# Robin-Lenoir/replication-social-bank-runs

Hardware: AMD Instinct MI355X
Metric: equilibria solved/sec on β×u grid (FP64) (higher is better)
Workload: dtype f64; 1 GPU; fig5_beta_u_sweep_2048x2048_per_gpu (BASELINE config 3); n_beta_per_gpu=2048, n_u=2048, early_exit=False, parallelism=beta-column shards x1, beta_axis_columns=2048, pipelined=True

## Files before the change

include/sbr.h:

```cpp
#ifndef SBR_H
#define SBR_H

#include <stdint.h>

#include "sbr_status.h"

#ifdef __cplusplus
extern "C" {
#endif

#define SBR_OK 0
#define SBR_EARG (-1)
#define SBR_EDEVICE (-2)
#define SBR_ENOMEM (-3)

typedef struct sbr_ctx sbr_ctx;

typedef struct {
    double ode_reltol;
    double ode_abstol;
    int64_t ode_maxiters;
    int32_t bisect_max_iters;
    int32_t early_exit_nan_run;
    int32_t knot_capacity;
    int32_t hetero_max_iters;
    int32_t flags;
    int32_t pad;
    double xi_guess;
} sbr_opts;

#define SBR_FLAG_EXHAUSTIVE 0x1
#define SBR_FLAG_READY_SWEEP 0x2
#define SBR_FLAG_RCCL_GATHER 0x4
#define SBR_FLAG_XI_GUESS 0x8
#define SBR_FLAG_DIAG_STOP_AFTER_BUFFER 0x100
#define SBR_FLAG_DIAG_STOP_AFTER_BISECT 0x200
#define SBR_FLAG_DIAG_COUNT_AW_BLOCKS 0x400
#define SBR_FLAG_DIAG_SOCIAL_PROF 0x800
#define SBR_FLAG_DIAG_NO_AW_WINDOW 0x1000
#define SBR_FLAG_HETERO_WIDE 0x2000

#define SBR_HETERO_MAX_K 16

typedef struct {
    double* xi;
    double* tau_in_unc;
    double* tau_out_unc;
    double* aw_max;
    double* tol;
    uint32_t* status;
    int32_t* iters;
} sbr_result_soa;

void sbr_default_opts(sbr_opts* o);

int sbr_init(int device, sbr_ctx** ctx);
int sbr_free(sbr_ctx* ctx);
const char* sbr_last_error(const sbr_ctx* ctx);

int sbr_init_multi(int n_gpus, const int* devices, sbr_ctx** ctx);
int sbr_multi_size(const sbr_ctx* ctx);
sbr_ctx* sbr_multi_child(sbr_ctx* ctx, int rank);

// ... 171 lines not shown
```

replication-social-bank-runs_amd/csrc/sbr_capi_baseline.hip:

```cpp
#include "sbr_hostio.h"

using namespace sbr_capi;

namespace sbr_capi {

void free_learn(sbr_ctx* c, int slot)
{
    sbr::LearnBufs& L = c->LW[slot];
    free_dev(L.t, L.G, L.hr, L.hrI, L.n_knots, L.n_tau, L.n_le, L.status, L.n_accept, L.n_reject);
    L = sbr::LearnBufs{};
    c->ws_beta[slot] = c->ws_cap[slot] = 0;
}

size_t learn_ld(size_t cap) { return ((cap + 15) & ~(size_t)15) + 16; }

int ensure_learn(sbr_ctx* c, size_t n_beta, size_t cap, int slot, bool hri)
{
    if (n_beta <= c->ws_beta[slot] && cap == c->ws_cap[slot] && (!hri || c->LW[slot].hrI)) return SBR_OK;
    free_learn(c, slot);
    sbr::LearnBufs& L = c->LW[slot];
    const size_t ld = learn_ld(cap);
    const size_t slab = n_beta * ld * sizeof(double);
    const int rc = alloc_dev(c, {{L.t, slab}, {L.G, slab}, {L.hr, slab}, {L.hrI, hri ? slab : 0},
                                 {L.n_knots, n_beta * 4}, {L.n_tau, n_beta * 4}, {L.n_le, n_beta * 4},
// ... 38 lines not shown
    free_econ(c);
    const int rc = alloc_dev(c, {{c->ec_hr, rows * ld * sizeof(double)}, {c->ec_cnt, rows * 3 * sizeof(int32_t)}});
    if (rc) return rc;
    c->ec_rows = rows;
    c->ec_ld = ld;
    return SBR_OK;
}

}

namespace {

int32_t stop_after_eta(const sbr_opts& o)
{
    const double e = 2.220446049250313e-16;
    return (o.ode_reltol == e && o.ode_abstol == e && o.ode_maxiters >= SBR_DEFAULT_ODE_MAXITERS) ? 1 : 0;
}

int launch_eq(sbr_ctx* c, hipStream_t s, const sbr::LearnBufs& L, const double* eta, const double* t_end,
              const double* u, int64_t n_beta, int64_t n_u, double kappa, const sbr_opts& o,
              const sbr::ResultSoA& out, double* aw_path, int group = 1, bool timed = true)
{
    sbr::EqArgs ea{kappa, (int32_t)n_u, o.bisect_max_iters, c->lds_cap_b, aw_path,
                   (o.flags & SBR_FLAG_EXHAUSTIVE) ? 1 : 0, (o.flags >> 8) & 0x17};
    ea.group = group;
    hipEvent_t t0 = timed ? tstart(c, s) : nullptr;
    if (aw_path && n_beta == 1 && n_u == 1) {
        ea.lds_cap = c->lds_cap;
        HIP_TRY(c, sbr::launch_point_coop(L, eta, t_end, u, ea, out, s), SBR_EDEVICE);
        tend(c, s, 1, t0);
        return SBR_OK;
    }
    HIP_TRY(c, sbr::launch_equilibrium(L, eta, t_end, u, ea, out, (int)n_beta, s), SBR_EDEVICE);
    tend(c, s, 1, t0);
    return SBR_OK;
}

#ifndef SBR_BATCH_LEARN_WAVES
#define SBR_BATCH_LEARN_WAVES 768
#endif
#ifndef SBR_BATCH_EQ_COLS
#define SBR_BATCH_EQ_COLS 4096
#endif
struct BatchPlan {
    int64_t L = 1;
    int64_t E = 1;
    int nslot = 1;
// ... 85 lines not shown
        c->rq_cap = need;
    }
    return SBR_OK;
}

int run_baseline_ready(sbr_ctx* c, hipStream_t s, const double* beta, const double* eta, const double* t_end,
                       const double* u, int64_t n_beta, int64_t n_u, double kappa, const sbr_opts& o,
                       sbr::LearnArgs la, const sbr::ResultSoA& out)
{
    const int tiles = (int)((n_u + kReadyTileU - 1) / kReadyTileU);
    int32_t* q = c->rq;
    HIP_TRY(c, hipEventRecord(c->ev_rin, s), SBR_EDEVICE);
    HIP_TRY(c, hipStreamWaitEvent(c->rs_learn, c->ev_rin, 0), SBR_EDEVICE);
    HIP_TRY(c, hipMemsetAsync(q, 0, (4 + 2 * (size_t)n_beta) * 4, c->rs_learn), SBR_EDEVICE);
    HIP_TRY(c, hipEventRecord(c->ev_rq, c->rs_learn), SBR_EDEVICE);
    HIP_TRY(c, hipStreamWaitEvent(c->rs_eq, c->ev_rq, 0), SBR_EDEVICE);
    la.fuse_hazard = 0;
    la.ready_tail = q + 2;
    la.ready_q = q + 4;
    hipEvent_t t0 = tstart(c, c->rs_learn);
    HIP_TRY(c, sbr::launch_learn_logistic(beta, eta, t_end, la, c->LW[0], c->rs_learn), SBR_EDEVICE);
    tend(c, c->rs_learn, 0, t0);
    sbr::EqArgs ea{kappa, (int32_t)n_u, o.bisect_max_iters, c->lds_cap_b, nullptr,
                   (o.flags & SBR_FLAG_EXHAUSTIVE) ? 1 : 0, (o.flags >> 8) & 0x17};
    sbr::ReadyArgs ra{q, q + 4, q + 4 + n_beta, (int32_t)(n_beta * tiles), tiles, kReadyTileU, kReadySpin};
    hipEvent_t t1 = tstart(c, c->rs_eq);
    HIP_TRY(c, sbr::launch_eq_ready(c->LW[0], beta, eta, t_end, u, la, ea, ra, out, 0, c->rs_eq), SBR_EDEVICE);
    tend(c, c->rs_eq, 1, t1);
    HIP_TRY(c, hipEventRecord(c->ev_rl, c->rs_learn), SBR_EDEVICE);
    HIP_TRY(c, hipEventRecord(c->ev_re, c->rs_eq), SBR_EDEVICE);
    HIP_TRY(c, hipStreamWaitEvent(s, c->ev_rl, 0), SBR_EDEVICE);
    HIP_TRY(c, hipStreamWaitEvent(s, c->ev_re, 0), SBR_EDEVICE);
    HIP_TRY(c, sbr::launch_ready_fail(q + 1, out, n_beta * n_u, s), SBR_EDEVICE);
    return SBR_OK;
}

int run_baseline(sbr_ctx* c, hipStream_t s, const double* beta, const double* eta, const double* t_end, double x0,
                 const double* u, int64_t n_beta, int64_t n_u, double p, double kappa, double lambda,
                 const sbr_opts& o, const sbr::ResultSoA& out, double* aw_path)
{
    int rc = ensure_learn(c, (size_t)n_beta, (size_t)o.knot_capacity);
    if (rc) return rc;
    c->last_slot = 0;
    c->last_off = 0;
    sbr::LearnArgs la{x0, o.ode_reltol, o.ode_abstol, p, lambda, o.ode_maxiters, (int32_t)n_beta, stop_after_eta(o), 0};
    c->rs_used = !aw_path && n_beta >= 64 && (o.flags & SBR_FLAG_READY_SWEEP) &&
                 ensure_ready(c, (size_t)n_beta) == SBR_OK;
// ... 14 lines not shown
        const int64_t wk = waves >> (kSweepChunks - k);
        lo[k] = std::min<int64_t>(n_beta, std::max<int64_t>(wk * 64, (int64_t)k * 64));
    }
    lo[1] = std::min<int64_t>(lo[2] - 64, std::max<int64_t>(64, (waves / kSweepFront) * 64));
    HIP_TRY(c, hipEventRecord(c->ev_in, s), SBR_EDEVICE);
    hipEvent_t t0 = tstart(c, s);
    c->ck_start = c->timing ? t0 : nullptr;
    c->ck_ev.assign(c->timing ? 2 * kSweepChunks : 0, nullptr);
    for (int k = 0; k < kSweepChunks; k++) {
        hipStream_t ls = c->lstream[k];
        const int64_t c0 = lo[k], nb = lo[k + 1] - lo[k];
        HIP_TRY(c, hipStreamWaitEvent(ls, c->ev_in, 0), SBR_EDEVICE);
        if (nb <= 0) continue;
        sbr::LearnArgs lk = la;
        lk.n_beta = (int32_t)nb;
        const sbr::LearnBufs Lk = learn_rows(c->LW[0], (size_t)c0);
        HIP_TRY(c, sbr::launch_learn_logistic(beta + c0, eta + c0, t_end + c0, lk, Lk, ls), SBR_EDEVICE);
        if (c->timing) {
            c->ck_ev[2 * k] = next_event(c);
            if (c->ck_ev[2 * k]) (void)hipEventRecord(c->ck_ev[2 * k], ls);
        }
        HIP_TRY(c, hipEventRecord(c->ev_learned[k], ls), SBR_EDEVICE);
        sbr::EqArgs ea{kappa, (int32_t)n_u, o.bisect_max_iters, c->lds_cap_b, nullptr,
                       (o.flags & SBR_FLAG_EXHAUSTIVE) ? 1 : 0, (o.flags >> 8) & 0x17};
        HIP_TRY(c, sbr::launch_equilibrium(Lk, eta + c0, t_end + c0, u, ea, result_rows(out, (size_t)(c0 * n_u)),
                                           (int)nb, ls), SBR_EDEVICE);
        if (c->timing) {
            c->ck_ev[2 * k + 1] = next_event(c);
            if (c->ck_ev[2 * k + 1]) (void)hipEventRecord(c->ck_ev[2 * k + 1], ls);
        }
        HIP_TRY(c, hipEventRecord(c->ev_eq[k], ls), SBR_EDEVICE);
    }
    for (int k = 0; k < kSweepChunks; k++)
        if (lo[k + 1] > lo[k]) HIP_TRY(c, hipStreamWaitEvent(s, c->ev_learned[k], 0), SBR_EDEVICE);
    hipEvent_t t1 = tstart(c, s);
    tend(c, s, 0, t0);
    for (int k = 0; k < kSweepChunks; k++)
        if (lo[k + 1] > lo[k]) HIP_TRY(c, hipStreamWaitEvent(s, c->ev_eq[k], 0), SBR_EDEVICE);
    tend(c, s, 1, t1);
    return SBR_OK;
}

size_t point_bytes(size_t cap) { return 4 * cap * sizeof(double) + 6 * sizeof(int32_t); }

int run_points(sbr_ctx* c, hipStream_t s, const double* beta, const double* eta, const double* t_end, double x0,
               const double* u, const double* p, const double* kappa, const double* lambda, int64_t n,
               const sbr_opts& o, const sbr::ResultSoA& out)
// ... 53 lines not shown
    const double budget = c->ec_budget > 0 ? (double)c->ec_budget : 0.4 * (double)(freeb + held);
    const double left = budget - (double)n_beta * (double)point_bytes(cap);
    int64_t per = left > 0.0 ? (int64_t)std::min(left / ((double)n_beta * (double)econ_class_bytes(cap)), 65535.0) : 1;
    per = std::max<int64_t>(1, std::min<int64_t>(per, n_class));
    int rc = ensure_learn(c, (size_t)n_beta, cap);
    if (rc) return rc;
    c->last_slot = 0;
    c->last_off = 0;
    c->rs_used = false;
    const sbr::LearnBufs& L = c->LW[0];
    for (;;) {
        rc = ensure_econ(c, (size_t)(per * n_beta), (size_t)L.cap);
        if (rc == SBR_OK) break;
        free_econ(c);
        if (per == 1) return rc;
        (void)hipGetLastError();
        per = (per + 1) / 2;
    }
    sbr::LearnArgs la{x0, o.ode_reltol, o.ode_abstol, 0.0, 0.0, o.ode_maxiters, (int32_t)n_beta, stop_after_eta(o), 0};
    hipEvent_t t0 = tstart(c, s);
    HIP_TRY(c, sbr::launch_learn_kernel(beta, eta, t_end, la, L, s, 1), SBR_EDEVICE);
    tend(c, s, 0, t0);
    sbr::EqArgs ea{0.0, (int32_t)(n_kappa * n_u), o.bisect_max_iters, rates ? c->lds_cap : c->lds_cap_b, nullptr,
                   (o.flags & SBR_FLAG_EXHAUSTIVE) ? 1 : 0, (o.flags >> 8) & 0x17};
    const sbr::InterestEconArgs ie{rates ? rates->r : nullptr, rates ? rates->delta : nullptr,
                                   (int32_t)(rates ? rates->n : 0), o.ode_reltol, o.ode_abstol, o.ode_maxiters,
                                   rates ? rates->steps : nullptr};
    t0 = tstart(c, s);
    int launches = 0;
    for (int64_t g0 = 0; g0 < n_class; g0 += per) {
        const int64_t ng = std::min<int64_t>(per, n_class - g0);
        const size_t rows = (size_t)(per * n_beta);
        const sbr::EconArgs e{p, lambda, kappa, (int32_t)n_p, (int32_t)n_lambda, (int32_t)n_kappa, (int32_t)n_u,
                              (int32_t)n_beta, (int32_t)g0, (int32_t)ng, c->ec_hr, c->ec_cnt, c->ec_cnt + rows,
                              (uint32_t*)(c->ec_cnt + 2 * rows)};
        HIP_TRY(c, sbr::launch_hazard_econ(beta, eta, la, L, e, s), SBR_EDEVICE);
        if (rates) HIP_TRY(c, sbr::launch_interest_econ(L, eta, t_end, u, ea, e, ie, out, s), SBR_EDEVICE);
        else HIP_TRY(c, sbr::launch_equilibrium_econ(L, eta, t_end, u, ea, e, out, s), SBR_EDEVICE);
        launches += 3;
    }
    tend(c, s, 1, t0, launches);
    return SBR_OK;
}

int econ_checks(sbr_ctx* c, const sbr_opts* opts, double x0, int64_t n_beta, int64_t n_u, int64_t n_p,
                int64_t n_lambda, int64_t n_kappa)
{
// ... 1 lines not shown
    if (!c) return SBR_EARG;
    const int64_t lim = 1 << 30;
    if (n_beta <= 0 || n_u <= 0 || n_p <= 0 || n_lambda <= 0 || n_kappa <= 0 || n_beta > lim || n_u > lim ||
        n_p > lim || n_lambda > lim || n_kappa > lim || n_p * n_lambda > lim || n_kappa * n_u > lim)
        return fail(c, SBR_EARG, "grid size");
    if (!(x0 >= 0.0)) return fail(c, SBR_EARG, "ArgumentError: x0");
    return SBR_OK;
}

int run_interest(sbr_ctx* c, hipStream_t s, const double* beta, const double* eta, const double* t_end, double x0,
                 const double* u, int64_t n_beta, int64_t n_u, double p, double kappa, double lambda, double r,
                 double delta, const sbr_opts& o, const sbr::ResultSoA& out, int64_t* steps, double* aw_path = nullptr,
                 double* v_path = nullptr, int32_t* v_count = nullptr)
{
    int rc = ensure_learn(c, (size_t)n_beta, (size_t)o.knot_capacity);
    if (rc) return rc;
    c->last_slot = 0;
    c->last_off = 0;
    sbr::LearnArgs la{x0, o.ode_reltol, o.ode_abstol, p, lambda, o.ode_maxiters, (int32_t)n_beta, stop_after_eta(o), 0};
    hipEvent_t t0 = tstart(c, s);
    HIP_TRY(c, sbr::launch_learn_logistic(beta, eta, t_end, la, c->LW[0], s), SBR_EDEVICE);
    tend(c, s, 0, t0);
    sbr::EqArgs ea{kappa, (int32_t)n_u, o.bisect_max_iters, c->lds_cap, aw_path,
                   (o.flags & SBR_FLAG_EXHAUSTIVE) ? 1 : 0, (o.flags >> 8) & 0x17};
    sbr::InterestArgs ia{r, delta, o.ode_reltol, o.ode_abstol, o.ode_maxiters, steps, v_path, v_count};
    t0 = tstart(c, s);
    HIP_TRY(c, sbr::launch_interest(c->LW[0], eta, t_end, u, ea, ia, out, (int)n_beta, s), SBR_EDEVICE);
    tend(c, s, 1, t0);
    return SBR_OK;
}

bool interest_valid(double r, double delta) { return r >= 0.0 && delta > 0.0 && r < delta; }

}

extern "C" {

int sbr_sweep_baseline_dev(sbr_ctx* c, void* stream, const double* beta, const double* eta, const double* t_end,
                           double x0, const double* u, int64_t n_beta, int64_t n_u, double p, double kappa,
                           double lambda, const sbr_opts* opts, sbr_result_soa* out)
{
    if (int rc = refuse_guess(c, opts)) return rc;
    SBR_SINGLE_DEVICE(c);
    if (!c || !has_fields(out)) return SBR_EARG;
    if (n_beta <= 0 || n_u <= 0 || n_beta > (1 << 30) || n_u > (1 << 30)) return fail(c, SBR_EARG, "grid size");
    if (!scalars_valid(x0, p, kappa, lambda)) return fail(c, SBR_EARG, "ArgumentError: x0/p/kappa/lambda");
    if (hipSetDevice(c->device) != hipSuccess) return fail(c, SBR_EDEVICE, "hipSetDevice");
// ... 643 lines not shown
```

replication-social-bank-runs_amd/csrc/sbr_capi_knots.hip:

```cpp
#include "sbr_hostio.h"

using namespace sbr_capi;

namespace {

struct KnotLayout {
    size_t sc, tg, hr, u, res, bytes;
    KnotLayout(size_t ck, size_t cu)
    {
        sc = 64;
        tg = 128;
        hr = tg + 24 * ck;
        u = hr + 8 * (ck + 8);
        res = u + 8 * (cu + 8);
        bytes = res + 8 * (6 * cu + 3 * (ck + 1)) + 256;
    }
};

int ensure_knots(sbr_ctx* c, size_t n, size_t n_u)
{
    if (n <= c->kn_cap_k && n_u <= c->kn_cap_u) return SBR_OK;
    size_t ck = c->kn_cap_k > 4096 ? c->kn_cap_k : 4096, cu = c->kn_cap_u > 64 ? c->kn_cap_u : 64;
    while (ck < n) ck *= 2;
    while (cu < n_u) cu *= 2;
// ... 246 lines not shown
            double* hs = (double*)(H + K.sc);
            hs[0] = beta;
            hs[1] = eta;
            memcpy(H + K.tg, t, (size_t)n * 8);
            memcpy(H + K.tg + (size_t)n * 8, G, (size_t)n * 8);
            if (pdf) memcpy(H + K.tg + (size_t)n * 16, pdf, (size_t)n * 8);
            HIP_TRY(c, hipMemcpyAsync(D, H, K.tg + (size_t)n * (pdf ? 24 : 16), hipMemcpyHostToDevice, s), SBR_EDEVICE);
            sbr::LearnArgs la{0.0, o.ode_reltol, o.ode_abstol, p, lambda, o.ode_maxiters, 1, 0, 0, nullptr, nullptr};
            la.pdf = pdf ? dtg + 2 * n : nullptr;
            HIP_TRY(c, sbr::launch_hazard(dsc, dsc + 1, la, L, 1, s), SBR_EDEVICE);
            if (ntau > 0)
                HIP_TRY(c, hipMemcpyAsync(H + K.hr, D + K.hr, (size_t)ntau * 8, hipMemcpyDeviceToHost, s), SBR_EDEVICE);
            HIP_TRY(c, hipMemcpyAsync(H, D, 32, hipMemcpyDeviceToHost, s), SBR_EDEVICE);
        }
        const size_t nu = (size_t)n_u;
        if (n_u == 1) {
            double* z = c->kn_zc;
            double* zd = c->kn_zc_dev;
            z[0] = t_end;
            z[1] = u[0];
            const sbr::ResultSoA r{zd + 2, zd + 3, zd + 4, zd + 5, zd + 6, (uint32_t*)(zd + 7), (int32_t*)(zd + 7) + 1};
            double* zp = zd + 16;
            sbr::EqArgs ea{kappa, 1, o.bisect_max_iters, c->lds_cap, want_aw ? zp : nullptr,
                           (o.flags & SBR_FLAG_EXHAUSTIVE) ? 1 : 0, (o.flags >> 8) & 0x17,
                           want_aw ? zp + ntau : nullptr, want_aw ? zp + 2 * ntau : nullptr, 1, dres};
            if (o.flags & SBR_FLAG_XI_GUESS) ea.xi_guess = o.xi_guess;
            HIP_TRY(c, sbr::launch_point_coop(L, dsc + 1, zd, zd + 1, ea, r, s), SBR_EDEVICE);
        } else {
            double* hu = (double*)(H + K.u);
            hu[0] = t_end;
            memcpy(hu + 1, u, nu * 8);
            HIP_TRY(c, hipMemcpyAsync(du, hu, (nu + 1) * 8, hipMemcpyHostToDevice, s), SBR_EDEVICE);
            const sbr::ResultSoA r{dres, dres + nu, dres + 2 * nu, dres + 3 * nu, dres + 4 * nu,
                                   (uint32_t*)(dres + 5 * nu), (int32_t*)(dres + 5 * nu) + nu};
            if ((o.flags & SBR_FLAG_XI_GUESS) && o.xi_guess == o.xi_guess) {
                sbr::EqArgs ea{kappa, 1, o.bisect_max_iters, c->lds_cap, nullptr,
                               (o.flags & SBR_FLAG_EXHAUSTIVE) ? 1 : 0, (o.flags >> 8) & 0x17, nullptr, nullptr, 1};
                ea.xi_guess = o.xi_guess;
                HIP_TRY(c, sbr::launch_point_coop(L, dsc + 1, du, du + 1, ea, r, s, (int)nu), SBR_EDEVICE);
            } else {
                sbr::EqArgs ea{kappa, (int32_t)n_u, o.bisect_max_iters, c->lds_cap_b, nullptr,
                               (o.flags & SBR_FLAG_EXHAUSTIVE) ? 1 : 0, (o.flags >> 8) & 0x17, nullptr, nullptr, 1};
                HIP_TRY(c, sbr::launch_equilibrium(L, dsc + 1, du, du + 1, ea, r, 1, s, n <= c->lds_cap_b ? 1 : 2),
                        SBR_EDEVICE);
            }
            HIP_TRY(c, hipMemcpyAsync(H + K.res, D + K.res, res_bytes, hipMemcpyDeviceToHost, s), SBR_EDEVICE);
        }
        HIP_TRY(c, hipStreamSynchronize(s), SBR_EDEVICE);
        return SBR_OK;
    });
    if (rc) return rc;
    if (!hit) {
        const int32_t* hc = (const int32_t*)H;
        if (hc[1] != (int32_t)ntau) return fail(c, SBR_EDEVICE, "hazard grid length mismatch");
        c->kn_t.assign(t, t + n);
        c->kn_G.assign(G, G + n);
        if (pdf) c->kn_pdf.assign(pdf, pdf + n);
        else c->kn_pdf.clear();
        const double* hh = (const double*)(H + K.hr);
        c->kn_hr.assign(hh, hh + ntau);
        memcpy(c->kn_key, key, sizeof key);
        c->kn_n = n;
        c->kn_m = (int32_t)m;
        c->kn_ntau = (int32_t)ntau;
        c->kn_valid = true;
// ... 50 lines not shown
```

replication-social-bank-runs_amd/csrc/sbr_eq_column_body.h:

```cpp
{
    const int n = L.n_knots[b], ntau = L.n_tau[b], nle = L.n_le[b];
    const uint32_t lst = L.status[b];
    const size_t row = (size_t)b * (size_t)L.cap;
    const double* __restrict__ gT = L.t + row;
    const double* __restrict__ gG = L.G + row;
    const double* __restrict__ gH = L.hr + row;
    constexpr int NS = INTEREST ? 3 : 2;
    const bool fits = n <= a.lds_cap && (!INTEREST || ntau <= a.lds_cap);
    if ((MODE == 1 && !fits) || (MODE == 2 && fits)) return;
    double* sT = smem;
    double* sG = smem + a.lds_cap;
    double* sH = INTEREST ? smem + 2 * a.lds_cap : nullptr;
    const double* __restrict__ cH = INTEREST ? sH : gH;
    const int nsum = (a.lds_cap >> 6) + 1, nsum8 = (a.lds_cap >> 3) + 1;
    double* hmax = smem + NS * a.lds_cap;
    double* hmin = hmax + nsum;
    double* pmc = hmin + nsum;
    double* smc = pmc + nsum8;
    double* hpm = smc + nsum8;
    double* hpn = hpm + nsum;
    double* hsm = hpn + nsum;
    double* hsn = hsm + nsum;
    const int nbh_s = (ntau + 63) >> 6;
    __shared__ int eq_next;
    __shared__ int s_nonmono;
    __shared__ int s_noscan;
    __shared__ int s_near1;
    __shared__ int s_ndec;
    __shared__ unsigned long long s_maxdec;
    __shared__ double s_thalf;
    __shared__ int s_wb;
    __shared__ unsigned long long s_dmax;
    if (threadIdx.x == 0) { eq_next = 0; s_nonmono = 0; s_noscan = 0; s_near1 = 0; s_ndec = 0; s_maxdec = 0; s_thalf = NAN; s_wb = 0x7fffffff; s_dmax = 0; }
    if (fits) {
        for (int i = threadIdx.x; i < n; i += BLOCK) { sT[i] = gT[i]; sG[i] = gG[i]; }
        if (INTEREST)
            for (int i = threadIdx.x; i < ntau; i += BLOCK) sH[i] = gH[i];
    }
    __syncthreads();
    Summ S{nullptr, nullptr, nullptr, nullptr, false, (double)NAN, false, 0.0, false, 2, nullptr, nullptr, nullptr,
           nullptr, 0};
    if (fits && !a.exhaustive) {
        const int nbh = (ntau + 63) >> 6, nbg = (n + 7) >> 3;
        const int nq = nbh << 3;
        for (int bk = threadIdx.x; bk < nq + nbg; bk += BLOCK) {
            if (bk < nq) {
                double mx = -INFINITY, mn = INFINITY;
                const int i0 = bk << 3;
                double h[8];
#pragma unroll
                for (int k = 0; k < 8; k++) h[k] = i0 + k < ntau ? cH[i0 + k] : -INFINITY;
#pragma unroll
                for (int k = 0; k < 8; k++) {
                    if (i0 + k >= ntau) continue;
                    if (h[k] > mx) mx = h[k];
                    mn = (h[k] != h[k]) ? -INFINITY : (h[k] < mn ? h[k] : mn);
// ... 15 lines not shown
                double prev = g > 0 ? sG[(g << 3) - 1] : -INFINITY;
                bool mono = true, nan = false;
                int ndec = 0;
                double maxdec = 0.0;
                for (int i = g << 3; i < e; i++) {
                    const double v = sG[i];
                    if (v != v) { mx = NAN; mn = NAN; mono = false; nan = true; break; }
                    if (v > mx) mx = v;
                    if (v < mn) mn = v;
                    const bool dec = v < prev;
                    mono &= !dec;
                    ndec += dec ? 1 : 0;
                    maxdec = dec && prev - v > maxdec ? prev - v : maxdec;
                    prev = v;
                }
                if (!mono) s_nonmono = 1;
                if (nan) s_noscan = 1;
                if (ndec) {
                    atomicAdd(&s_ndec, ndec);
                    atomicMax(&s_maxdec, (unsigned long long)sbr_dbits(maxdec));
                }
                const double sep = 1e-15 * sT[n - 1];
                bool far = true, far1 = true;
                for (int i = g << 3; i < e; i++) {
                    far &= i + 2 >= n || sT[i + 2] - sT[i] > sep;
                    far1 &= i + 1 >= n || sT[i + 1] - sT[i] > sep;
                }
                if (!far) s_noscan = 1;
                if (!far1) s_near1 = 1;
                pmc[g] = mx;
                smc[g] = mn;
            }
        }
        {
            auto rises = [](double lo, double hi) {
                const double m = fabs(lo) > fabs(hi) ? fabs(lo) : fabs(hi);
                return m >= 0x1p-900 && m <= 1e300 && hi - lo > 0x1p-50 * m;
            };
            const int ln = threadIdx.x & 63;
            for (int q = threadIdx.x >> 6; q * 62 < n - 1; q += BLOCK >> 6) {
                const int k = q * 62 + ln - 2;
                const bool valid = k >= 0 && k <= n - 2;
                const double d = valid ? (sG[k + 1] - sG[k]) / (sT[k + 1] - sT[k]) : 0.0;
                const double d1 = __shfl_up(d, 1, 64);
                const bool inc = rises(d1, d), dec = rises(d, d1);
                const bool incp = __shfl_up((int)inc, 1, 64) != 0;
                const bool mine = valid && ln >= 2;
                const bool fail = mine && k >= 1 && ((!inc && !dec) || (k >= 2 && inc && !incp));
                double ad = mine ? fabs(d) : 0.0;
                ad = ad <= 1e300 ? ad : (double)INFINITY;
#pragma unroll
                for (int off = 1; off < 64; off <<= 1) {
// ... 74 lines not shown
            const unsigned long long v = sbr_dbits(x);
            const unsigned lo = __builtin_amdgcn_readfirstlane((unsigned)v);
            const unsigned hi = __builtin_amdgcn_readfirstlane((unsigned)(v >> 32));
            return sbr_bitsd(((unsigned long long)hi << 32) | lo);
        };
        const double dd = uni((double)s_ndec * sbr_bitsd(s_maxdec));
        S = Summ{hmax, hmin, pmc, smc, s_nonmono == 0, uni(s_thalf),
                 n >= 2 && !s_noscan && dd <= 1e-12 && sG[0] >= 0.0 && sG[n - 1] <= 2.0, dd,
                 s_nonmono == 0 || s_noscan != 0, s_near1 == 0 ? 1 : 2,
                 hpm, hpn, hsm, hsn, nbh_s};
        const double dmax = sbr_bitsd(s_dmax);
        if (n >= 2 && dmax <= 1e300 && !(a.diag & 16)) {
            const int wb = s_wb < n - 1 ? s_wb : n - 1;
            const double e0 = fabs(sT[0]), e1 = fabs(sT[n - 1]);
            const double span = (sT[wb] + 2.0 * (e0 > e1 ? e0 : e1)) * (1.0 + 0x1p-40);
            const double du = 0x1p-52 * span;
            const double wm = 0x1p-46 + dmax * (0x1p-50 * span);
            if (wm <= 1e-9) {
                S.wlo = uni((sT[0] > 0.0 ? sT[0] : 0.0) + du);
                S.whi = uni(sT[wb] - du);
                S.wm = uni(wm);
            }
        }
    }
    const int lane = threadIdx.x & 63;
    const double ETA = eta[b], T1 = t_end[b];
    const uint32_t lbits = lst & (SBR_ODE_MAXITERS | SBR_STIFF_SWITCH | SBR_ODE_FAILED | SBR_KNOT_OVERFLOW);
    const bool bad_col = (lst & (SBR_ARG_INVALID | SBR_OOB)) || n < 2;
    const bool trunc = !a.full_grid && n >= 2 && gT[n - 1] < T1 && !(lst & kLearnCutBits);
    for (;;) {
        int base = 0;
        if (lane == 0) base = atomicAdd(&eq_next, 64);
        base = __builtin_amdgcn_readfirstlane(base);
        if (j0 + base >= j1) break;
        const int j = j0 + base + lane;
        if (j >= j1) continue;
#ifdef SBR_EQ_LANE
        SBR_EQ_LANE(j);
#else
        const double uj = SBR_EQ_U(j);
        PointResult r;
        int64_t vsteps = 0;
        if (bad_col || SBR_EQ_BAD(uj, j)) {
            r.xi = NAN; r.aw = NAN; r.tol = INFINITY; r.iters = 0;
            r.tin = NAN; r.tout = NAN;
            r.status = ((lst & SBR_ARG_INVALID) || SBR_EQ_BAD(uj, j)) ? SBR_ARG_INVALID : (SBR_OOB | lbits);
// ... 26 lines not shown
```

replication-social-bank-runs_amd/csrc/sbr_eq_dev.h:

```cpp
#pragma once

#include "sbr_device.h"
#include "sbr_hazard_dev.h"
#include "sbr_kernels.h"
#include "sbr_ode.h"
#include "sbr_scan.h"
#include "sbr_solve_dev.h"

namespace sbr {

template <class P>
__device__ __forceinline__ void solve_point(P T, P G, P H, const Summ& S, const int n, const int ntau,
                                            const int nle, const double ETA, const double T1, const bool trunc,
                                            const double u, const double kappa, const int max_iters,
                                            const uint32_t lbits, PointResult& r, double* __restrict__ aw_path,
                                            const int diag)
{
    r.xi = NAN; r.aw = NAN; r.tol = INFINITY; r.iters = 0; r.status = 0;
    (void)0;

    bool any, all;
    int fa, la, cin, cout;
    if (S.hpm) {
        buffer_scan_bs(H, S, S.hpm, S.hpn, S.hsm, S.hsn, S.nbh, ntau, u, any, all, fa, la, cin, cout);
// ... 112 lines not shown
            const bool oke = in_range(xoe, tlo, thi, trunc, flag);
            const bool oki = in_range(xie, tlo, thi, trunc, flag);
            if (flag) break;
            const double AW = Goc - Gic;
            const double err = AW - kappa;
            if (fabs(err) <= tolerance) {
                double Goce = 0.0, Gice = 0.0;
                if (oke) Goce = lerp_at(T, G, n, ssl_gallop(T, n, joc, xoe), xoe);
                if (oki) Gice = lerp_at(T, G, n, ssl_gallop(T, n, jic, xie), xie);
                const double AWe = Goce - Gice;
                if (AWe >= AW) { s = SBR_RUN; xi = xo; tolr = fabs(err); }
                else s = SBR_FALSE_EQ;
                break;
            } else if (err > 0) {
                xmax = xo; jhi = j; xnew = 0.5 * (xo + xmin);
            } else {
                xmin = xo; jlo = j; xnew = 0.5 * (xo + xmax);
            }
            const bool inside = ORD || (moderate && ic == tin && tin <= xmin && xmax <= tout);
            single = single || (inside && jlo == jhi && xmax + eps <= thi && eps > 0.0);
            if (__ballot(!single) == 0) { live = true; iter++; break; }
        }
    };
    if (__ballot(!(moderate && tin <= tout)) == 0) loop_a(BoolC<true>{});
    else loop_a(BoolC<false>{});
    if (live) {
        const int j = jlo;
        const double t0 = T[j], g0 = G[j], g1 = G[j + 1], eps = T[j + 1] - t0, Gic = c_ic_v;
        const bool rcp_ok = eps >= 0x1p-64 && eps <= 0x1p64 &&
                            (fabs(t0) >= 0x1p-840 || (t0 == 0.0 && xmin >= 0x1p-900));
        const bool use_rcp = __ballot(!rcp_ok) == 0;
        const double rinv = rcp_refined(eps);
        const int last = max_iters - 1;
        int ex = 0;
        double xo = xnew, err = 0.0, Goc = 0.0;
        auto trips = [&](auto quot) {
            for (; iter <= max_iters; iter++) {
                r.iters = iter;
                const bool col = collapsed(xmin - xmax);
                xo = xnew;
                const double d = quot(xo - t0);
                Goc = g0 * (1.0 - d) + g1 * d;
                err = (Goc - Gic) - kappa;
                const bool ter = fabs(err) <= tolerance;
                if (col || iter == last || ter) { ex = col ? 1 : (iter == last ? 2 : 3); break; }
                const bool up = err > 0;
                const double other = up ? xmin : xmax;
                xmax = up ? xo : xmax;
                xmin = up ? xmin : xo;
                xnew = 0.5 * (xo + other);
            }
        };
        if (use_rcp) trips([&](double a) { return div_rcp(a, eps, rinv); });
        else trips([&](double a) { return a / eps; });
        if (ex == 1) s = SBR_NO_RUN_COLLAPSE;
        else if (ex == 3) {
            const double xoe = xo + eps, xie = tin + eps, AW = Goc - Gic;
            const double Goce = lerp_at(T, G, n, ssl_gallop(T, n, j, xoe), xoe);
            const double Gice = lerp_at(T, G, n, ssl_gallop(T, n, jtin, xie), xie);
            if (Goce - Gice >= AW) { s = SBR_RUN; xi = xo; tolr = fabs(err); }
            else s = SBR_FALSE_EQ;
        }
    }
    if (flag) { r.status = flag | lbits; return; }
    if (s != SBR_RUN) { r.status = s | lbits; return; }
    if (diag & 2) return;
    int nblk_eval = 0;

    const double icc = (tin >= xi) ? xi : tin;
    const double occ = (tout > xi) ? xi : tout;
    if (!in_range(0.0, tlo, thi, trunc, flag)) { r.status = flag | lbits; return; }
    const double G0 = lerp_at(T, G, n, ssl_range(T, 0, n - 1, 0.0), 0.0);
    double mx = -INFINITY;
    auto xa_of = [&](int i) { const double v = (tau(i) - xi) + icc; return v > 0 ? v : 0.0; };
    auto xb_of = [&](int i) { const double v = (tau(i) - xi) + occ; return v > 0 ? v : 0.0; };
    int ra_i = 0, ra_j = 0, rb_i = 0, rb_j = 0;
    auto brk_a = [&](int i) { ra_j = ssl_near(T, n, ra_j + (i - ra_i), xa_of(i)); ra_i = i; return ra_j; };
    auto brk_b = [&](int i) { rb_j = ssl_near(T, n, rb_j + (i - rb_i), xb_of(i)); rb_i = i; return rb_j; };
    auto eval_range = [&](int i0, int i1) {
        int ka = brk_a(i0), kb = brk_b(i0);
        ka = ka < n - 2 ? ka : n - 2;
        kb = kb < n - 2 ? kb : n - 2;
        double ta0 = T[ka], ta1 = T[ka + 1], ga0 = G[ka], ga1 = G[ka + 1];
        double tb0 = T[kb], tb1 = T[kb + 1], gb0 = G[kb], gb1 = G[kb + 1];
        for (int i = i0; i < i1; i++) {
            const double ti = tau(i);
// ... 22 lines not shown
    const double tstar = S.t_half + 0.5 * ((xi - icc) + (xi - occ));
    const bool predicted = tstar == tstar && tstar >= tau(0) && tstar <= tau(ntau - 1);
    const bool scan = S.scan && predicted;
    if (!S.pmc || aw_path || !(scan || S.bnb)) {
        eval_range(0, ntau);
    } else {
        const double al = (tau(ntau - 1) - xi) + icc, bl = (tau(ntau - 1) - xi) + occ;
        if (!((al > 0 ? al : 0.0) <= thi) || !((bl > 0 ? bl : 0.0) <= thi)) {
            flag |= trunc ? SBR_ENGINE_TRUNC : SBR_OOB;
        } else {
            auto ub_rng = [&](int i0, int i1) -> double {
                const int ja = brk_a(i0), jb = brk_b(i1);
                const int kh = jb + 1 < n - 1 ? jb + 1 : n - 1, kl = ja < n - 2 ? ja : n - 2;
                const double hi = S.mono ? G[kh] : S.pmc[kh >> 3];
                const double lo = S.mono ? G[kl] : S.smc[kl >> 3];
                const double ub_out = hi > 0.0 ? hi : 0.0;
                const double lb_in = ((tau(i0) - xi) + icc) >= 0 ? lo : (lo < 0.0 ? lo : 0.0);
                return ((ub_out - lb_in) + G0) + 1e-14;
            };
            auto end_of = [&](int i0, int w) { return i0 + w < ntau ? i0 + w : ntau; };
            const int ic = predicted ? ssl_range(T, 0, (nle > 0 ? nle : 1) - 1, tstar < T[0] ? T[0] : tstar) : 0;
            if (scan) {
                aw_scan(T, G, n, ntau, nle, ETA, xi, icc, occ, G0, S.dd, ic < ntau ? ic : ntau - 1, mx, nblk_eval,
                        S.koff, S.wlo, S.whi, S.wm);
            } else
            {
            int b8 = -1, w0 = 0, w1 = 0;
            if (predicted) {
                const int c8 = (ic < ntau ? ic : ntau - 1) & ~7;
                w0 = c8 - 8 * kAwWin > 0 ? c8 - 8 * kAwWin : 0;
                w1 = end_of(c8, 8 * (kAwWin + 1));
                eval_range(w0, w1);
            } else {
                int bs = 0;
                double bu = -INFINITY;
                for (int i0 = 0; i0 < ntau; i0 += 256) {
                    const double ub = ub_rng(i0, end_of(i0, 256) - 1);
                    if (!(ub <= bu)) { bu = ub; bs = i0; }
                }
                int bb = bs;
                bu = -INFINITY;
                for (int i0 = bs; i0 < end_of(bs, 256); i0 += 64) {
                    const double ub = ub_rng(i0, end_of(i0, 64) - 1);
                    if (!(ub <= bu)) { bu = ub; bb = i0; }
                }
                b8 = bb;
                bu = -INFINITY;
// ... 253 lines not shown
```

replication-social-bank-runs_amd/csrc/sbr_solve_dev.h:

```cpp
#pragma once

#include "sbr_device.h"
#include "sbr_kernels.h"
#include "sbr_scan.h"
#include "sbr_hazard_dev.h"

namespace sbr {

struct PointResult {
    double xi, tin, tout, aw, tol;
    uint32_t status;
    int iters;
};

constexpr uint32_t kLearnCutBits = SBR_ODE_MAXITERS | SBR_KNOT_OVERFLOW | SBR_ODE_FAILED;

__device__ __forceinline__ bool in_range(double x, double tlo, double thi, bool trunc, uint32_t& flag)
{
    if (x >= tlo && x <= thi) return true;
    flag |= (trunc && x > thi) ? SBR_ENGINE_TRUNC : SBR_OOB;
    return false;
}

struct Summ {
    const double* hmax;
    const double* hmin;
    const double* pmc;
    const double* smc;
    bool mono;
    double t_half;
    bool scan;
    double dd;
    bool bnb;
    int koff;
    const double* hpm;
    const double* hpn;
    const double* hsm;
    const double* hsn;
    int nbh;
    double wlo = INFINITY, whi = -INFINITY, wm = 0.0;
};

template <class P>
__device__ __forceinline__ void solve_from_buffers(P T, P G, P H, const Summ& S, const int n, const int ntau,
                                                   const int nle, const double ETA, const double T1, const bool trunc,
                                                   const double u, const double kappa, const int max_iters,
                                                   const uint32_t lbits, PointResult& r, double* __restrict__ aw_path,
                                                   const int diag, const double tin, const double tout);

template <class F>
__device__ __forceinline__ int first_ge_down(F key, int hi, double x)
{
    int top = hi, lo = hi - 1, step = 1;
    while (lo >= 0 && key(lo) >= x) {
        top = lo;
        step <<= 1;
        lo = top - step;
    }
    if (lo < -1) lo = -1;
    while (top - lo > 1) {
        const int mid = (lo + top) >> 1;
        if (key(mid) >= x) top = mid;
        else lo = mid;
    }
    return top;
}

template <class P>
__device__ __forceinline__ void aw_scan(P T, P G, const int n, const int ntau, const int nle, const double ETA,
                                        const double xi, const double icc, const double occ, const double G0,
                                        const double dd, const int c, double& mx, int& nev, const int koff = 2,
                                        const double wlo = INFINITY, const double whi = -INFINITY,
                                        const double wm = 0.0)
{
    const double M = 1e-14 + 4.0 * dd;
    const double Mw = M + wm;
    const bool wuse = occ >= icc && wlo <= whi;
    auto tau = [&](int i) -> double { return i < nle ? T[i] : ETA; };
    auto bv_of = [&](int i) -> double { return (tau(i) - xi) + occ; };
    auto av_of = [&](int i) -> double { return (tau(i) - xi) + icc; };
    int ka;
    double ta0, ta1, ga0, ga1;
    auto seek = [&](int hint, double x) {
        ka = ssl_near(T, n, hint, x);
        ka = ka < n - 2 ? ka : n - 2;
        ta0 = T[ka]; ta1 = T[ka + 1]; ga0 = G[ka]; ga1 = G[ka + 1];
    };
    auto fwd = [&](double x) {
        while (ka < n - 2 && ta1 <= x) { ka++; ta0 = ta1; ga0 = ga1; ta1 = T[ka + 1]; ga1 = G[ka + 1]; }
    };
    auto bwd = [&](double x) {
        while (ka > 0 && ta0 > x) { ka--; ta1 = ta0; ga1 = ga0; ta0 = T[ka]; ga0 = G[ka]; }
    };
    double awin = 0.0, awout = 0.0;
    auto exact = [&](int i, double av, double xa) -> double {
        const double ti = tau(i);
        const double bv = (ti - xi) + occ;
        const double xb = bv > 0 ? bv : 0.0;
        int kb = (i < nle && xb == ti) ? i : ssl_near(T, n, i, xb);
// ... 154 lines not shown
```

replication-social-bank-runs_amd/sbr/_lib.py:

```python
from __future__ import annotations

import ctypes
import os
import re
from pathlib import Path

PKG_ROOT = Path(__file__).resolve().parent.parent
REPO_ROOT = PKG_ROOT.parent
LIB_PATH = Path(os.environ["SBR_LIB"]) if os.environ.get("SBR_LIB") else PKG_ROOT / "lib" / "libsbr.so"
HEADER = REPO_ROOT / "include" / "sbr.h"
STATUS_HEADER = REPO_ROOT / "include" / "sbr_status.h"

_D = ctypes.c_double
_I64 = ctypes.c_int64
_I32 = ctypes.c_int32
_P = ctypes.c_void_p

SBR_OK, SBR_EARG, SBR_EDEVICE, SBR_ENOMEM = 0, -1, -2, -3
SBR_FLAG_EXHAUSTIVE = 0x1
SBR_FLAG_READY_SWEEP = 0x2
SBR_FLAG_RCCL_GATHER = 0x4
SBR_FLAG_XI_GUESS = 0x8
SBR_FLAG_DIAG_STOP_AFTER_BUFFER = 0x100
SBR_FLAG_DIAG_STOP_AFTER_BISECT = 0x200
SBR_FLAG_DIAG_COUNT_AW_BLOCKS = 0x400
SBR_FLAG_DIAG_SOCIAL_PROF = 0x800
SBR_FLAG_DIAG_NO_AW_WINDOW = 0x1000
SBR_FLAG_HETERO_WIDE = 0x2000
SBR_HETERO_MAX_K = 16


class SBRNativeError(RuntimeError):
    """The native engine is unavailable or returned an error."""


class ArgumentError(ValueError):
    """Mirror of Julia's ArgumentError raised by the reference's constructors."""


class Opts(ctypes.Structure):
    _fields_ = [
        ("ode_reltol", _D),
        ("ode_abstol", _D),
        ("ode_maxiters", _I64),
        ("bisect_max_iters", _I32),
        ("early_exit_nan_run", _I32),
        ("knot_capacity", _I32),
        ("hetero_max_iters", _I32),
        ("flags", _I32),
        ("pad", _I32),
        ("xi_guess", _D),
# ... 149 lines not shown
```

Before: 6.032 billion equilibria/s.

## Pre-decide bisection bracket with knot-gap test to skip segment search loop

Result: slower. 5.816 billion equilibria/s (-3.6%).

```diff
diff --git a/include/sbr.h b/include/sbr.h
--- a/include/sbr.h
+++ b/include/sbr.h
@@ -39,6 +39,8 @@
 #define SBR_FLAG_DIAG_SOCIAL_PROF 0x800
 #define SBR_FLAG_DIAG_NO_AW_WINDOW 0x1000
 #define SBR_FLAG_HETERO_WIDE 0x2000
+#define SBR_FLAG_DIAG_NO_REGLOOP 0x4000
+#define SBR_FLAG_DIAG_COUNT_DECIDED 0x8000
 
 #define SBR_HETERO_MAX_K 16
 
diff --git a/replication-social-bank-runs_amd/csrc/sbr_capi_baseline.hip b/replication-social-bank-runs_amd/csrc/sbr_capi_baseline.hip
--- a/replication-social-bank-runs_amd/csrc/sbr_capi_baseline.hip
+++ b/replication-social-bank-runs_amd/csrc/sbr_capi_baseline.hip
@@ -84,7 +84,7 @@
               const sbr::ResultSoA& out, double* aw_path, int group = 1, bool timed = true)
 {
     sbr::EqArgs ea{kappa, (int32_t)n_u, o.bisect_max_iters, c->lds_cap_b, aw_path,
-                   (o.flags & SBR_FLAG_EXHAUSTIVE) ? 1 : 0, (o.flags >> 8) & 0x17};
+                   (o.flags & SBR_FLAG_EXHAUSTIVE) ? 1 : 0, (o.flags >> 8) & 0xd7};
     ea.group = group;
     hipEvent_t t0 = timed ? tstart(c, s) : nullptr;
     if (aw_path && n_beta == 1 && n_u == 1) {
@@ -216,7 +216,7 @@
     HIP_TRY(c, sbr::launch_learn_logistic(beta, eta, t_end, la, c->LW[0], c->rs_learn), SBR_EDEVICE);
     tend(c, c->rs_learn, 0, t0);
     sbr::EqArgs ea{kappa, (int32_t)n_u, o.bisect_max_iters, c->lds_cap_b, nullptr,
-                   (o.flags & SBR_FLAG_EXHAUSTIVE) ? 1 : 0, (o.flags >> 8) & 0x17};
+                   (o.flags & SBR_FLAG_EXHAUSTIVE) ? 1 : 0, (o.flags >> 8) & 0xd7};
     sbr::ReadyArgs ra{q, q + 4, q + 4 + n_beta, (int32_t)(n_beta * tiles), tiles, kReadyTileU, kReadySpin};
     hipEvent_t t1 = tstart(c, c->rs_eq);
     HIP_TRY(c, sbr::launch_eq_ready(c->LW[0], beta, eta, t_end, u, la, ea, ra, out, 0, c->rs_eq), SBR_EDEVICE);
@@ -277,7 +277,7 @@
         }
         HIP_TRY(c, hipEventRecord(c->ev_learned[k], ls), SBR_EDEVICE);
         sbr::EqArgs ea{kappa, (int32_t)n_u, o.bisect_max_iters, c->lds_cap_b, nullptr,
-                       (o.flags & SBR_FLAG_EXHAUSTIVE) ? 1 : 0, (o.flags >> 8) & 0x17};
+                       (o.flags & SBR_FLAG_EXHAUSTIVE) ? 1 : 0, (o.flags >> 8) & 0xd7};
         HIP_TRY(c, sbr::launch_equilibrium(Lk, eta + c0, t_end + c0, u, ea, result_rows(out, (size_t)(c0 * n_u)),
                                            (int)nb, ls), SBR_EDEVICE);
         if (c->timing) {
@@ -377,7 +377,7 @@
     HIP_TRY(c, sbr::launch_learn_kernel(beta, eta, t_end, la, L, s, 1), SBR_EDEVICE);
     tend(c, s, 0, t0);
     sbr::EqArgs ea{0.0, (int32_t)(n_kappa * n_u), o.bisect_max_iters, rates ? c->lds_cap : c->lds_cap_b, nullptr,
-                   (o.flags & SBR_FLAG_EXHAUSTIVE) ? 1 : 0, (o.flags >> 8) & 0x17};
+                   (o.flags & SBR_FLAG_EXHAUSTIVE) ? 1 : 0, (o.flags >> 8) & 0xd7};
     const sbr::InterestEconArgs ie{rates ? rates->r : nullptr, rates ? rates->delta : nullptr,
                                    (int32_t)(rates ? rates->n : 0), o.ode_reltol, o.ode_abstol, o.ode_maxiters,
                                    rates ? rates->steps : nullptr};
@@ -425,7 +425,7 @@
     HIP_TRY(c, sbr::launch_learn_logistic(beta, eta, t_end, la, c->LW[0], s), SBR_EDEVICE);
     tend(c, s, 0, t0);
     sbr::EqArgs ea{kappa, (int32_t)n_u, o.bisect_max_iters, c->lds_cap, aw_path,
-                   (o.flags & SBR_FLAG_EXHAUSTIVE) ? 1 : 0, (o.flags >> 8) & 0x17};
+                   (o.flags & SBR_FLAG_EXHAUSTIVE) ? 1 : 0, (o.flags >> 8) & 0xd7};
     sbr::InterestArgs ia{r, delta, o.ode_reltol, o.ode_abstol, o.ode_maxiters, steps, v_path, v_count};
     t0 = tstart(c, s);
     HIP_TRY(c, sbr::launch_interest(c->LW[0], eta, t_end, u, ea, ia, out, (int)n_beta, s), SBR_EDEVICE);
diff --git a/replication-social-bank-runs_amd/csrc/sbr_capi_knots.hip b/replication-social-bank-runs_amd/csrc/sbr_capi_knots.hip
--- a/replication-social-bank-runs_amd/csrc/sbr_capi_knots.hip
+++ b/replication-social-bank-runs_amd/csrc/sbr_capi_knots.hip
@@ -292,7 +292,7 @@
             const sbr::ResultSoA r{zd + 2, zd + 3, zd + 4, zd + 5, zd + 6, (uint32_t*)(zd + 7), (int32_t*)(zd + 7) + 1};
             double* zp = zd + 16;
             sbr::EqArgs ea{kappa, 1, o.bisect_max_iters, c->lds_cap, want_aw ? zp : nullptr,
-                           (o.flags & SBR_FLAG_EXHAUSTIVE) ? 1 : 0, (o.flags >> 8) & 0x17,
+                           (o.flags & SBR_FLAG_EXHAUSTIVE) ? 1 : 0, (o.flags >> 8) & 0xd7,
                            want_aw ? zp + ntau : nullptr, want_aw ? zp + 2 * ntau : nullptr, 1, dres};
             if (o.flags & SBR_FLAG_XI_GUESS) ea.xi_guess = o.xi_guess;
             HIP_TRY(c, sbr::launch_point_coop(L, dsc + 1, zd, zd + 1, ea, r, s), SBR_EDEVICE);
@@ -305,12 +305,12 @@
                                    (uint32_t*)(dres + 5 * nu), (int32_t*)(dres + 5 * nu) + nu};
             if ((o.flags & SBR_FLAG_XI_GUESS) && o.xi_guess == o.xi_guess) {
                 sbr::EqArgs ea{kappa, 1, o.bisect_max_iters, c->lds_cap, nullptr,
-                               (o.flags & SBR_FLAG_EXHAUSTIVE) ? 1 : 0, (o.flags >> 8) & 0x17, nullptr, nullptr, 1};
+                               (o.flags & SBR_FLAG_EXHAUSTIVE) ? 1 : 0, (o.flags >> 8) & 0xd7, nullptr, nullptr, 1};
                 ea.xi_guess = o.xi_guess;
                 HIP_TRY(c, sbr::launch_point_coop(L, dsc + 1, du, du + 1, ea, r, s, (int)nu), SBR_EDEVICE);
             } else {
                 sbr::EqArgs ea{kappa, (int32_t)n_u, o.bisect_max_iters, c->lds_cap_b, nullptr,
-                               (o.flags & SBR_FLAG_EXHAUSTIVE) ? 1 : 0, (o.flags >> 8) & 0x17, nullptr, nullptr, 1};
+                               (o.flags & SBR_FLAG_EXHAUSTIVE) ? 1 : 0, (o.flags >> 8) & 0xd7, nullptr, nullptr, 1};
                 HIP_TRY(c, sbr::launch_equilibrium(L, dsc + 1, du, du + 1, ea, r, 1, s, n <= c->lds_cap_b ? 1 : 2),
                         SBR_EDEVICE);
             }
diff --git a/replication-social-bank-runs_amd/csrc/sbr_eq_column_body.h b/replication-social-bank-runs_amd/csrc/sbr_eq_column_body.h
--- a/replication-social-bank-runs_amd/csrc/sbr_eq_column_body.h
+++ b/replication-social-bank-runs_amd/csrc/sbr_eq_column_body.h
@@ -31,7 +31,8 @@
     __shared__ double s_thalf;
     __shared__ int s_wb;
     __shared__ unsigned long long s_dmax;
-    if (threadIdx.x == 0) { eq_next = 0; s_nonmono = 0; s_noscan = 0; s_near1 = 0; s_ndec = 0; s_maxdec = 0; s_thalf = NAN; s_wb = 0x7fffffff; s_dmax = 0; }
+    __shared__ unsigned long long s_gs;
+    if (threadIdx.x == 0) { eq_next = 0; s_nonmono = 0; s_noscan = 0; s_near1 = 0; s_ndec = 0; s_maxdec = 0; s_thalf = NAN; s_wb = 0x7fffffff; s_dmax = 0; s_gs = 0; }
     if (fits) {
         for (int i = threadIdx.x; i < n; i += BLOCK) { sT[i] = gT[i]; sG[i] = gG[i]; }
         if (INTEREST)
@@ -93,12 +94,16 @@
                 }
                 const double sep = 1e-15 * sT[n - 1];
                 bool far = true, far1 = true;
+                const double eta_b = eta[b];
+                double gsl = 0.0;
                 for (int i = g << 3; i < e; i++) {
                     far &= i + 2 >= n || sT[i + 2] - sT[i] > sep;
                     far1 &= i + 1 >= n || sT[i + 1] - sT[i] > sep;
+                    if (i + 1 < n && sT[i] <= eta_b && sT[i + 1] - sT[i] > gsl) gsl = sT[i + 1] - sT[i];
                 }
                 if (!far) s_noscan = 1;
                 if (!far1) s_near1 = 1;
+                if (gsl > 0.0) atomicMax(&s_gs, (unsigned long long)sbr_dbits(gsl));
                 pmc[g] = mx;
                 smc[g] = mn;
             }
@@ -219,6 +224,12 @@
                 S.wm = uni(wm);
             }
         }
+        const bool regloop = S.scan && s_near1 == 0 && sT[n - 1] > 0.0 && sT[0] >= -0x1p1000 && sT[n - 1] <= 0x1p1000 &&
+                             !(a.diag & 64);
+        S.gs = uni(regloop ? sbr_bitsd(s_gs) : (double)INFINITY);
+        S.bm = uni(1e-13 + 4.0 * dd);
+        S.am = uni(1e-14 + 4.0 * dd);
+        S.amw = uni((1e-14 + 4.0 * dd) + S.wm);
     }
     const int lane = threadIdx.x & 63;
     const double ETA = eta[b], T1 = t_end[b];
diff --git a/replication-social-bank-runs_amd/csrc/sbr_eq_dev.h b/replication-social-bank-runs_amd/csrc/sbr_eq_dev.h
--- a/replication-social-bank-runs_amd/csrc/sbr_eq_dev.h
+++ b/replication-social-bank-runs_amd/csrc/sbr_eq_dev.h
@@ -158,11 +158,39 @@
             if (__ballot(!single) == 0) { live = true; iter++; break; }
         }
     };
-    if (__ballot(!(moderate && tin <= tout)) == 0) loop_a(BoolC<true>{});
-    else loop_a(BoolC<false>{});
+    bool qual = false, allneg = false, allpos = false;
+    if (S.gs < (double)INFINITY) {
+        if (tin <= tout && tout < thi && tout <= ETA && tolerance <= 1e-14 && tout + S.gs <= thi) {
+            c_ic_v = lerp_at(T, G, n, jtin, tin);
+            const double tgt = c_ic_v + kappa;
+            const double below = tgt - S.bm, above = tgt + S.bm;
+            const double gl = G[jtin], gh = G[jhi + 1];
+            if (gh <= below) qual = allneg = true;
+            else if (gl >= above) qual = allpos = true;
+            else if (gl <= below) {
+                int hi = jhi + 1;
+                while (hi - jlo > 1) {
+                    const int mid = (jlo + hi) >> 1;
+                    if (G[mid] <= below) jlo = mid;
+                    else hi = mid;
+                }
+                qual = G[jlo + 1] >= above;
+            }
+        }
+    }
+    if (__ballot(!qual) == 0) live = true;
+    else {
+        jlo = jtin;
+        allneg = allpos = false;
+        if (__ballot(!(moderate && tin <= tout)) == 0) loop_a(BoolC<true>{});
+        else loop_a(BoolC<false>{});
+    }
+    int ndec = 0;
     if (live) {
         const int j = jlo;
-        const double t0 = T[j], g0 = G[j], g1 = G[j + 1], eps = T[j + 1] - t0, Gic = c_ic_v;
+        const double g0 = G[j], g1 = G[j + 1], eps = T[j + 1] - T[j], Gic = c_ic_v;
+        const double t0 = allneg ? (double)INFINITY : allpos ? -(double)INFINITY : T[j];
+        const double t1 = allneg ? (double)INFINITY : allpos ? -(double)INFINITY : T[j + 1];
         const bool rcp_ok = eps >= 0x1p-64 && eps <= 0x1p64 &&
                             (fabs(t0) >= 0x1p-840 || (t0 == 0.0 && xmin >= 0x1p-900));
         const bool use_rcp = __ballot(!rcp_ok) == 0;
@@ -170,7 +198,7 @@
         const int last = max_iters - 1;
         int ex = 0;
         double xo = xnew, err = 0.0, Goc = 0.0;
-        auto trips = [&](auto quot) {
+        auto trips = [&](auto quot, auto count) {
             for (; iter <= max_iters; iter++) {
                 r.iters = iter;
                 const bool col = collapsed(xmin - xmax);
@@ -178,17 +206,23 @@
                 const double d = quot(xo - t0);
                 Goc = g0 * (1.0 - d) + g1 * d;
                 err = (Goc - Gic) - kappa;
-                const bool ter = fabs(err) <= tolerance;
+                const bool lt = xo < t0, ge = xo >= t1;
+                const bool ter = !(lt | ge) & (fabs(err) <= tolerance);
                 if (col || iter == last || ter) { ex = col ? 1 : (iter == last ? 2 : 3); break; }
-                const bool up = err > 0;
+                const bool up = ge | (!lt & (err > 0));
+                if constexpr (decltype(count)::value) ndec += (lt | ge) ? 1 : 0;
                 const double other = up ? xmin : xmax;
                 xmax = up ? xo : xmax;
                 xmin = up ? xmin : xo;
                 xnew = 0.5 * (xo + other);
             }
         };
-        if (use_rcp) trips([&](double a) { return div_rcp(a, eps, rinv); });
-        else trips([&](double a) { return a / eps; });
+        auto run = [&](auto count) {
+            if (use_rcp) trips([&](double a) { return div_rcp(a, eps, rinv); }, count);
+            else trips([&](double a) { return a / eps; }, count);
+        };
+        if (diag & 128) run(BoolC<true>{});
+        else run(BoolC<false>{});
         if (ex == 1) s = SBR_NO_RUN_COLLAPSE;
         else if (ex == 3) {
             const double xoe = xo + eps, xie = tin + eps, AW = Goc - Gic;
@@ -198,6 +232,7 @@
             else s = SBR_FALSE_EQ;
         }
     }
+    if (diag & 128) r.iters = ndec;
     if (flag) { r.status = flag | lbits; return; }
     if (s != SBR_RUN) { r.status = s | lbits; return; }
     if (diag & 2) return;
@@ -266,7 +301,7 @@
             const int ic = predicted ? ssl_range(T, 0, (nle > 0 ? nle : 1) - 1, tstar < T[0] ? T[0] : tstar) : 0;
             if (scan) {
                 aw_scan(T, G, n, ntau, nle, ETA, xi, icc, occ, G0, S.dd, ic < ntau ? ic : ntau - 1, mx, nblk_eval,
-                        S.koff, S.wlo, S.whi, S.wm);
+                        S.koff, S.wlo, S.whi, S.am, S.amw);
             } else
             {
             int b8 = -1, w0 = 0, w1 = 0;
diff --git a/replication-social-bank-runs_amd/csrc/sbr_solve_dev.h b/replication-social-bank-runs_amd/csrc/sbr_solve_dev.h
--- a/replication-social-bank-runs_amd/csrc/sbr_solve_dev.h
+++ b/replication-social-bank-runs_amd/csrc/sbr_solve_dev.h
@@ -39,6 +39,9 @@
     const double* hsn;
     int nbh;
     double wlo = INFINITY, whi = -INFINITY, wm = 0.0;
+    double gs = INFINITY;
+    double bm = INFINITY;
+    double am = 1e-14, amw = 1e-14;
 };
 
 template <class P>
@@ -69,12 +72,9 @@
 template <class P>
 __device__ __forceinline__ void aw_scan(P T, P G, const int n, const int ntau, const int nle, const double ETA,
                                         const double xi, const double icc, const double occ, const double G0,
-                                        const double dd, const int c, double& mx, int& nev, const int koff = 2,
-                                        const double wlo = INFINITY, const double whi = -INFINITY,
-                                        const double wm = 0.0)
-{
-    const double M = 1e-14 + 4.0 * dd;
-    const double Mw = M + wm;
+                                        const double dd, const int c, double& mx, int& nev, const int koff,
+                                        const double wlo, const double whi, const double M, const double Mw)
+{
     const bool wuse = occ >= icc && wlo <= whi;
     auto tau = [&](int i) -> double { return i < nle ? T[i] : ETA; };
     auto bv_of = [&](int i) -> double { return (tau(i) - xi) + occ; };
diff --git a/replication-social-bank-runs_amd/sbr/_lib.py b/replication-social-bank-runs_amd/sbr/_lib.py
--- a/replication-social-bank-runs_amd/sbr/_lib.py
+++ b/replication-social-bank-runs_amd/sbr/_lib.py
@@ -27,6 +27,8 @@
 SBR_FLAG_DIAG_SOCIAL_PROF = 0x800
 SBR_FLAG_DIAG_NO_AW_WINDOW = 0x1000
 SBR_FLAG_HETERO_WIDE = 0x2000
+SBR_FLAG_DIAG_NO_REGLOOP = 0x4000
+SBR_FLAG_DIAG_COUNT_DECIDED = 0x8000
 SBR_HETERO_MAX_K = 16
 
 
```
